# spaceandtimefdn/blitzar

Hardware: NVIDIA H100
Metric: MSM throughput (scalar*point terms/sec), ristretto255, n=2^20 per GPU (higher is better)
Workload: dtype u32 limbs (integer modular arithmetic)

## Files before the change

blitzar_b200/csrc/msm.cuh:

```cuda
#pragma once
#include <algorithm>
#include <vector>

#include "batch_affine.cuh"
#include "curve.cuh"
#include "engine_api.cuh"
#include "lanefield.cuh"

namespace b200 {

struct ColumnDesc {
  const unsigned char* base;
  u64 row_stride;
  u32 bit_offset;
  u32 bit_width;
  u32 n;
  u32 is_signed;
  u32 first_window;
  u32 num_windows;
  u32 table_n;
  u32 gen_base;
};
B200_HD u32 bucket_windows(const ColumnDesc& col) { return col.table_n ? (col.num_windows ? 1u : 0u) : col.num_windows; }

// ... 832 lines not shown
    typename F::E prefix[kMaxTableWindows], acc = F::one(), inv;
    C::gen_to_point(p, table[i], false);
    for (u32 w = 0; w < W; ++w) {
      if (w)
        for (u32 k = 0; k < c; ++k)
          C::dbl(p, p);
      pts[w] = p;
      prefix[w] = acc;
      F::mul(acc, acc, C::denominator(p));
    }
    F::invert(inv, acc);
    for (u32 w = W; w-- > 0;) {
      typename F::E zi;
      F::mul(zi, inv, prefix[w]);
      F::mul(inv, inv, C::denominator(pts[w]));
      typename C::Gen g;
      C::normalized_gen(g, pts[w], zi);
      table[(u64)w * n + i] = g;
    }
  }
};
template <class C> struct IngestCompactBody {
  static constexpr int kBlock = 128;
  const unsigned char* table;
  u32 window_width;
  typename C::Gen* gens;
  B200_HD void operator()(u64 i) const {
    const u64 group = i / window_width, j = i % window_width;
    const u64 entry = (group << window_width) + (1ull << j);
    typename C::Gen g;
    C::load_compact_abi(g, table + entry * C::kAbiCompactBytes);
    gens[i] = g;
  }
};
struct BuiltinGeneratorBody {
  static constexpr int kBlock = 64;
  Ed25519::Gen* gens;
  u64 first;
  B200_HD void operator()(u64 i) const {
    Ed25519::Point g;
    Ed25519::builtin_generator(g, first + i);
    Ed25519::point_to_gen(gens[i], g);
  }
};
struct GenPieces {
  const u64* start;
  const u64* from;
  const u64* to;
  u32 npieces;
};
template <class C> struct IngestPiecesBody {
  static constexpr int kBlock = IngestBody<C, false>::kBlock;
  const unsigned char* raw;
  typename C::Gen* gens;
  GenPieces p;
  B200_HD void operator()(u64 tid) const {
    const u32 k = column_of(p.start, p.npieces, tid);
    IngestBody<C, false>{raw + p.from[k] * C::kAbiGenBytes, gens + p.to[k]}(tid - p.start[k]);
  }
};
struct BuiltinPiecesBody {
  static constexpr int kBlock = BuiltinGeneratorBody::kBlock;
  Ed25519::Gen* gens;
  GenPieces p;
  B200_HD void operator()(u64 tid) const {
    const u32 k = column_of(p.start, p.npieces, tid);
    BuiltinGeneratorBody{gens + p.to[k], p.from[k]}(tid - p.start[k]);
  }
};

struct IngestMap {
  GenPieces p;
  B200_HD void at(u64 i, u64& src, u64& dst) const {
    if (p.npieces == 0) {
      src = dst = i;
      return;
    }
    const u32 k = column_of(p.start, p.npieces, i);
    src = p.from[k] + (i - p.start[k]);
    dst = p.to[k] + (i - p.start[k]);
  }
};
constexpr u32 kNormBlock = 256;
struct NormalizeUpBody {
  static constexpr int kBlock = 128;
  typedef F25519 F;
  const unsigned char* raw;
  IngestMap map;
  u64 n, T;
  F::E* pre;
  F::E* prod;
  u32* invalid;
  B200_HD F::E group(u64 j) const {
    F::E z[kBatchGroup], acc = F::one();
#pragma unroll
    for (u32 k = 0; k < kBatchGroup; ++k) {
      const u64 i = j + k * T;
      z[k] = F::one();
      if (i < n) {
        u64 src, dst;
        map.at(i, src, dst);
        z[k] = Ed25519::load_abi_z(raw + src * Ed25519::kAbiGenBytes);
      }
    }
#pragma unroll
    for (u32 k = 0; k < kBatchGroup; ++k) {
      const u64 i = j + k * T;
      if (i >= n)
        break;
      if (F::is_zero(z[k])) {
        *invalid = 1u;
        z[k] = F::one();
      }
      pre[i] = acc;
      F::mul(acc, acc, z[k]);
    }
    return acc;
  }
  B200_HD void operator()(u64 j) const { prod[j] = group(j); }
};
struct NormalizeDownBody {
  static constexpr int kBlock = 128;
  typedef F25519 F;
  const unsigned char* raw;
  IngestMap map;
  u64 n, T;
  const F::E* pre;
  const F::E* prod;
  const F::E* ps;
  const u32* invalid;
  Ed25519::Gen* gens;
  B200_HD void operator()(u64 j) const {
    const bool scale = *invalid == 0;
    F::E inv = prod[ps ? j / kNormBlock : j];
    if (ps)
      F::mul(inv, inv, ps[j]);
    for (u32 k = kBatchGroup; k-- > 0;) {
      const u64 i = j + k * T;
      if (i >= n)
        continue;
      u64 src, dst;
      map.at(i, src, dst);
      Ed25519::Point p;
      Ed25519::load_point_abi(p, raw + src * Ed25519::kAbiGenBytes);
      if (scale) {
        F::E zi;
        F::mul(zi, inv, pre[i]);
        F::mul(inv, inv, p.Z);
        F::mul(p.X, p.X, zi);
        F::mul(p.Y, p.Y, zi);
        F::mul(p.T, p.T, zi);
        p.Z = F::one();
      }
      Ed25519::Gen g;
      Ed25519::point_to_gen(g, p);
      gens[dst] = g;
    }
  }
};
#ifdef B200_BINNED_SORT
__device__ __forceinline__ F25519::E shfl_up_fe(const F25519::E& a, u32 d) {
  F25519::E r;
#pragma unroll
  for (int k = 0; k < 8; ++k)
    r.l[k] = __shfl_up_sync(0xffffffffu, a.l[k], d);
  return r;
}
__device__ __forceinline__ F25519::E shfl_down_fe(const F25519::E& a, u32 d) {
  F25519::E r;
#pragma unroll
  for (int k = 0; k < 8; ++k)
    r.l[k] = __shfl_down_sync(0xffffffffu, a.l[k], d);
  return r;
}
template <int kBlock>
__device__ void block_prefix_suffix(const F25519::E& x, F25519::E& P, F25519::E& S,
                                    F25519::E& total, F25519::E* ws) {
  typedef F25519 F;
  const u32 lane = threadIdx.x & 31u, warp = threadIdx.x >> 5;
  F::E inc = x, sinc = x;
#pragma unroll
  for (u32 d = 1; d < 32; d <<= 1) {
    const F::E y = shfl_up_fe(inc, d), z = shfl_down_fe(sinc, d);
    if (lane >= d)
      F::mul(inc, inc, y);
    if (lane + d < 32)
      F::mul(sinc, sinc, z);
  }
  F::E pe = shfl_up_fe(inc, 1), se = shfl_down_fe(sinc, 1);
  if (lane == 0)
    pe = F::one();
  if (lane == 31) {
    se = F::one();
    ws[warp] = inc;
  }
  __syncthreads();
  F::E before = F::one(), after = F::one();
  for (u32 w = 0; w < kBlock / 32; ++w) {
    if (w < warp)
      F::mul(before, before, ws[w]);
    else if (w > warp)
      F::mul(after, after, ws[w]);
  }
  F::mul(P, before, pe);
  F::mul(S, se, after);
  F::mul(total, before, ws[warp]);
  F::mul(total, total, after);
  __syncthreads();
}
struct NormalizeUpBlockBody {
  static constexpr int kBlock = kNormBlock;
  typedef F25519 F;
  NormalizeUpBody up;
  F::E* ps;
  F::E* prod;
  __device__ void run(u32 b, unsigned char*) const {
    __shared__ F::E ws[kBlock / 32];
    const u64 j = (u64)b * kBlock + threadIdx.x;
    const F::E g = j < up.T ? up.group(j) : F::one();
    F::E P, S, total;
    block_prefix_suffix<kBlock>(g, P, S, total, ws);
    if (j < up.T)
      F::mul(ps[j], P, S);
    if (threadIdx.x == 0)
      prod[b] = total;
  }
};
struct NormalizeMidBody {
  static constexpr int kBlock = 1024;
  typedef F25519 F;
  F::E* vals;
  F::E* pre;
  u64 m;
  __device__ void run(u32, unsigned char*) const {
    __shared__ F::E ws[kBlock / 32];
    __shared__ F::E inv_total;
    const u64 per = (m + kBlock - 1) / kBlock, lo = min((u64)threadIdx.x * per, m),
              hi = min(lo + per, m);
    F::E c = F::one();
    for (u64 k = lo; k < hi; ++k) {
      pre[k] = c;
      F::mul(c, c, vals[k]);
    }
    F::E P, S, total;
    block_prefix_suffix<kBlock>(c, P, S, total, ws);
    if (threadIdx.x == 0)
      F::invert(inv_total, total);
    __syncthreads();
    F::E inv;
    F::mul(inv, inv_total, P);
    F::mul(inv, inv, S);
    for (u64 k = hi; k-- > lo;) {
      const F::E v = vals[k];
      F::mul(vals[k], inv, pre[k]);
      F::mul(inv, inv, v);
    }
  }
};
#endif
inline void ingest_normalized(stream_t s, const unsigned char* raw, Ed25519::Gen* gens,
                              const IngestMap& map, u64 n, u32* invalid) {
  typedef F25519::E fe;
  if (n == 0)
    return;
  const u64 T = (n + kBatchGroup - 1) / kBatchGroup;
  fe* pre = (fe*)dev_alloc(n * sizeof(fe), s);
  const NormalizeUpBody up{raw, map, n, T, pre, nullptr, invalid};
#ifdef B200_BINNED_SORT
  const u64 blocks = (T + kNormBlock - 1) / kNormBlock;
  fe* ps = (fe*)dev_alloc((T + 2 * blocks) * sizeof(fe), s);
  fe* prod = ps + T;
  launch_blocks(NormalizeUpBlockBody{up, ps, prod}, blocks, 0, s);
  launch_blocks(NormalizeMidBody{prod, prod + blocks, blocks}, 1, 0, s);
  launch(NormalizeDownBody{raw, map, n, T, pre, prod, ps, invalid, gens}, T, s);
  dev_free(ps, s);
#else
  fe* prod = (fe*)dev_alloc(T * sizeof(fe), s);
  NormalizeUpBody u = up;
  u.prod = prod;
  launch(u, T, s);
  batch_invert<F25519>(s, prod, T);
  launch(NormalizeDownBody{raw, map, n, T, pre, prod, nullptr, invalid, gens}, T, s);
  dev_free(prod, s);
#endif
  dev_free(pre, s);
}
template <class C, bool kCommit> struct StoreBody {
  static constexpr int kBlock = 32;
  const typename C::Point* pts;
  unsigned char* out;
  B200_HD void operator()(u64 i) const {
    if (kCommit)
      C::store_commit_abi(out + i * C::kAbiCommitBytes, pts[i]);
    else
      C::store_proj_abi(out + i * C::kAbiProjBytes, pts[i]);
  }
};
template <class C>
inline void launch_store_commit(stream_t s, const typename C::Point* pts, unsigned char* out,
                                u64 count, bool lane_tail) {
#ifdef B200_LANE_TAIL
  if constexpr (C::kCurveId == kRistretto255) {
    if (lane_tail && count && count <= 4096) {
      launch(StoreLaneBody{pts, out, count}, (count + 2) / 3 * 32, s);
      return;
    }
  }
#endif
  launch(StoreBody<C, true>{pts, out}, count, s);
}
template <class C> struct GenToProjBody {
  static constexpr int kBlock = 64;
  const typename C::Gen* gens;
  unsigned char* out;
  B200_HD void operator()(u64 i) const {
    typename C::Point p;
    C::gen_to_point(p, gens[i], false);
    C::store_proj_abi(out + i * C::kAbiProjBytes, p);
  }
};
template <class C> struct SumPartsBody {
  static constexpr int kBlock = 32;
  const typename C::Point* parts;
  u32 nparts, count;
  typename C::Point* out;
  B200_HD void operator()(u64 j) const {
    typename C::Point acc = parts[j];
    for (u32 r = 1; r < nparts; ++r)
      C::add(acc, acc, parts[(u64)r * count + j]);
    out[j] = acc;
  }
};

inline u32 choose_window_bits(u64 max_n, u32 max_width, u32 ncols, size_t point_bytes) {
  const double kMaxBucketBytes = 3.0e9;
  u32 best = 2;
  double best_cost = 1e300;
  for (u32 c = 2; c <= 16; ++c) {
    double W = (double)(max_width / c + 1);
    if (c > 8 && W * (double)(1u << (c - 1)) * (double)ncols * (double)point_bytes > kMaxBucketBytes)
      break;
    double cost = W * ((double)max_n + 2.5 * (double)(1u << (c - 1)));
    if (cost < best_cost) {
      best_cost = cost;
      best = c;
    }
  }
  return best;
}

struct MsmPlan {
  u32 c = 0, nbuckets = 0, ncols = 0, total_windows = 0;
  u64 nkeys = 0, max_n = 0, total_terms = 0, total_entries = 0;
  std::vector<ColumnDesc> cols;
};

inline MsmPlan msm_make_plan(std::vector<ColumnDesc> cols, const MsmOptions& opt,
                             size_t point_bytes) {
  MsmPlan p;
  p.ncols = (u32)cols.size();
  u32 max_width = 1;
  for (auto& col : cols) {
    p.max_n = std::max<u64>(p.max_n, col.n);
    p.total_terms += col.n;
    if (col.n)
      max_width = std::max(max_width, col.bit_width);
  }
  p.c = opt.window_bits ? opt.window_bits
                        : choose_window_bits(p.max_n, max_width, p.ncols, point_bytes);
  p.nbuckets = 1u << (p.c - 1);
  u64 max_entries = 0;
  for (auto& col : cols) {
    col.first_window = p.total_windows;
    col.num_windows = col.n ? col.bit_width / p.c + 1 : 0;
    p.total_windows += bucket_windows(col);
    max_entries += (u64)col.n * col.num_windows;
    if (col.table_n)
      B200_REQUIRE((u64)col.table_n * col.num_windows < (1ull << 31), "generator table too large");
    if (col.n)
      B200_REQUIRE((u64)col.gen_base + col.n + (u64)(col.num_windows - 1) * col.table_n < (1ull << 31),
                   "generator index of a column too large");
  }
  p.nkeys = (u64)p.total_windows * p.nbuckets;
  p.total_entries = max_entries;
  B200_REQUIRE(p.nkeys < (1ull << 32), "too many buckets for one pass");
  p.cols = std::move(cols);
  return p;
}

struct StagedRange {
  const ColumnDesc* d_cols = nullptr;
  const u64* d_col_start = nullptr;
  u64 total_terms = 0, max_entries = 0;
  u32 max_windows = 0;
  StagedRange(stream_t s, const MsmPlan& plan, u64 begin, u64 end) {
    const u32 ncols = plan.ncols;
    std::vector<ColumnDesc> cols(plan.cols);
    std::vector<u64> col_start(ncols + 1, 0);
    for (u32 j = 0; j < ncols; ++j) {
      u64 lo = std::min<u64>(begin, cols[j].n), hi = std::min<u64>(end, cols[j].n);
      cols[j].base += lo * cols[j].row_stride;
      cols[j].n = (u32)(hi - lo);
      col_start[j + 1] = col_start[j] + cols[j].n;
      max_entries += (u64)cols[j].n * cols[j].num_windows;
      max_windows = std::max(max_windows, cols[j].n ? cols[j].num_windows : 0u);
    }
    total_terms = col_start[ncols];
    if (total_terms == 0)
      return;
    B200_REQUIRE(max_entries < (1ull << 32) && end - begin < (1ull << 31),
                 "too many (term, window) entries for one sort pass");
    const size_t desc_bytes = ncols * sizeof(ColumnDesc), start_bytes = (ncols + 1) * sizeof(u64);
    std::vector<unsigned char> stage(desc_bytes + start_bytes);
    std::memcpy(stage.data(), cols.data(), desc_bytes);
    std::memcpy(stage.data() + desc_bytes, col_start.data(), start_bytes);
    d_cols = (const ColumnDesc*)stage_to_device(s, stage.data(), stage.size());
    d_col_start = (const u64*)((const unsigned char*)d_cols + desc_bytes);
  }
};

struct SortedLayout {
  u64* entries;
  u32* counts;
  u32* starts;
  u32* d_m;
  u64 slots_max;
  bool binned;
  BucketOffsets offsets() const { return {counts, starts}; }
};

inline SortedLayout sort_entries(stream_t s, const MsmPlan& plan, const StagedRange& r, u32 L,
                                 const MsmOptions& opt, u32* window_used) {
  const u32 ncols = plan.ncols, c = plan.c, nbuckets = plan.nbuckets;
  const u64 nkeys = plan.nkeys, max_entries = r.max_entries, total_terms = r.total_terms;
  SortedLayout out{};
  out.slots_max = L ? ((max_entries + nkeys * ((1ull << L) - 1) + (1ull << L) - 1) >> L) << L : max_entries;
  out.counts = (u32*)dev_alloc((nkeys + 1) * sizeof(u32), s);
  out.d_m = (u32*)dev_alloc(16 * sizeof(u32), s);
  out.entries = (u64*)dev_alloc(out.slots_max * sizeof(u64), s);
#ifdef B200_BINNED_SORT
  out.binned = L == 0 && opt.sort_path != 0 && binned_sort_shift(nkeys) <= kMaxBinShift &&
               (opt.sort_path == 2 || max_entries >= kBinnedSortMinEntries);
  if (out.binned)
    binned_sort(s, r.d_cols, r.d_col_start, ncols, c, nbuckets, total_terms, max_entries,
                r.max_windows, nkeys, out.entries, out.counts, out.d_m);
#endif
  if (!out.binned) {
    dev_zero(out.counts, (nkeys + 1) * sizeof(u32), s);
    launch(CountBody{r.d_cols, r.d_col_start, ncols, c, nbuckets, out.counts}, total_terms, s);
    if (L)
      launch(PadCountsBody{out.counts, (1u << L) - 1u}, nkeys, s);
    exclusive_scan(out.counts, nkeys + 1, s);
    copy_d2d(out.d_m, out.counts + nkeys, sizeof(u32), s);
    if (L) {
      out.starts = (u32*)dev_alloc((nkeys + 1) * sizeof(u32), s);
      copy_d2d(out.starts, out.counts, (nkeys + 1) * sizeof(u32), s);
    }
    const bool window_major = opt.scatter_window_major && r.max_windows > 1;
    launch(ScatterBody{r.d_cols, r.d_col_start, ncols, c, nbuckets, out.counts, out.entries,
                       window_major ? total_terms : 0},
           window_major ? total_terms * r.max_windows : total_terms, s);
  }
  if (L)
    launch(FillPadsBody{out.starts, out.counts, out.entries}, nkeys, s);
  launch(WindowUsedBody{out.offsets(), nbuckets, window_used}, plan.total_windows, s);
  return out;
}

inline unsigned sort_selftest(stream_t s, std::vector<ColumnDesc> cols, u32 c) {
  MsmOptions opt;
  opt.window_bits = c;
  const MsmPlan plan = msm_make_plan(std::move(cols), opt, 160);
  const StagedRange r(s, plan, 0, plan.max_n);
  if (r.total_terms == 0)
    return ~0u;
  const u64 nkeys = plan.nkeys, M = r.max_entries;
  DevBuf<u32> window_used(plan.total_windows, s);
  opt.sort_path = 0;
  const SortedLayout a = sort_entries(s, plan, r, 0, opt, window_used.p);
  opt.sort_path = 2;
  const SortedLayout b = sort_entries(s, plan, r, 0, opt, window_used.p);
  std::vector<u32> ca(nkeys + 1), cb(nkeys + 1), m(1);
  std::vector<u64> ea(M), eb(M);
  copy_d2h(ca.data(), a.counts, (nkeys + 1) * sizeof(u32), s);
  copy_d2h(cb.data(), b.counts, (nkeys + 1) * sizeof(u32), s);
  copy_d2h(m.data(), b.d_m, sizeof(u32), s);
  copy_d2h(ea.data(), a.entries, M * sizeof(u64), s);
  copy_d2h(eb.data(), b.entries, M * sizeof(u64), s);
  stream_sync(s);
  for (void* p : {(void*)a.entries, (void*)a.counts, (void*)a.d_m, (void*)b.entries, (void*)b.counts,
                  (void*)b.d_m, (void*)r.d_cols})
    dev_free(p, s);
  if (!b.binned)
    return ~0u;
  unsigned bad = m[0] == ca[nkeys] ? 0u : 1u;
  for (u64 k = 0; k < nkeys; ++k) {
    const u32 lo = k ? ca[k - 1] : 0u, hi = ca[k];
    if (cb[k] != hi || hi < lo || hi > M) {
      ++bad;
      continue;
    }
    std::sort(ea.begin() + lo, ea.begin() + hi);
    std::sort(eb.begin() + lo, eb.begin() + hi);
    if (!std::equal(ea.begin() + lo, ea.begin() + hi, eb.begin() + lo))
      ++bad;
  }
  return bad;
}

struct RangeHook {
  virtual void before_range(u64 begin, u64 end) = 0;
  virtual void before_accumulate() {}
  virtual ~RangeHook() {}
};

template <class C>
stream_t chunk_walk(stream_t s, stream_t tail, WalkInput<C> walk, u32* d_m, bool unit,
                    const u32* unit_veto, typename C::Point* target, const MsmOptions& opt,
                    std::vector<void*>& to_free) {
  typedef typename C::Point Point;
  u32 K = opt.chunk1 ? std::max(opt.chunk1, 4u) : (walk.m_max >= (1ull << 23) ? 64u : 32u);
  const u32 chunkn = std::max(opt.chunkn, 4u);
  const u32* lvl_keys = nullptr;
  const Point* lvl_pieces = nullptr;
  stream_t cs = s;
  for (int level = 0;; ++level) {
    const bool final_level = walk.m_max <= K;
    u64 T = (walk.m_max + K - 1) / K;
    u32* out_keys = final_level ? nullptr : (u32*)dev_alloc(2 * T * sizeof(u32), cs);
    Point* out_pieces = final_level ? nullptr : (Point*)dev_alloc(2 * T * sizeof(Point), cs);
    to_free.insert(to_free.end(), {out_keys, out_pieces});
    u32* out_m = d_m + 1 + (level % 8);
    const auto launch_level = [&](auto body, u64 threads, stream_t st) {
      body = {lvl_keys, walk.entries, walk.gens, lvl_pieces, walk.m_ptr, K, final_level, target,
              out_keys, out_pieces, out_m, unit_veto};
      launch(body, threads, st);
    };
    if (level == 0) {
      const bool uniform =
          opt.uniform_add == 2 ? C::kCurveId == kRistretto255 : opt.uniform_add != 0;
      constexpr bool kEd = C::kCurveId == kRistretto255;
      const bool unit_path = kEd && unit;
      if (uniform && unit_path)
        launch_level(AccumulateBody<C, true, SeqExec, true, kEd>{}, T, s);
      else if (uniform)
        launch_level(AccumulateBody<C, true, SeqExec, true>{}, T, s);
      else if (unit_path)
        launch_level(AccumulateBody<C, true, SeqExec, false, kEd>{}, T, s);
      else
        launch_level(AccumulateBody<C, true>{}, T, s);
      KernelTimer::get().end(s);
      if (tail != s)
        stream_follow(tail, s);
      cs = tail;
    } else if (T <= opt.quad_threshold) {
      launch_level(AccumulateBody<C, false, QuadExec>{}, T * QuadExec::kLanes, cs);
    } else {
      launch_level(AccumulateBody<C, false>{}, T, cs);
    }
    if (final_level)
      break;
    lvl_keys = out_keys;
    lvl_pieces = out_pieces;
    walk.m_ptr = out_m;
    walk.m_max = 2 * T;
    K = chunkn;
  }
  return cs;
}

template <class C>
void msm_accumulate_range(stream_t s, const MsmPlan& plan, const typename C::Gen* gens, u64 begin,
                          u64 end, bool add_into, typename C::Point* d_buckets,
                          u32* d_window_used, const MsmOptions& opt, stream_t tail,
                          RangeHook* hook = nullptr) {
  const StagedRange r(s, plan, begin, end);
  if (r.total_terms == 0)
    return;
  gens += begin;
  StageRange nvtx_sort("msm: digit count + scan + scatter");
  const u64 max_entries = r.max_entries, nkeys = plan.nkeys;
  u32 L = 0;
  if constexpr (C::kBatchAffine) {
    const double mean = (double)max_entries / (double)nkeys;
    if (opt.pair_levels >= 0)
      L = (u32)opt.pair_levels;
    else if (max_entries >= (1ull << 23))
      while (L < 6 && (double)(32u << L) <= mean)
        ++L;
    while (L > 0 && max_entries + nkeys * ((1ull << L) - 1) >= (1ull << 32) - (1ull << L))
      --L;
  }
  const SortedLayout sorted = sort_entries(s, plan, r, L, opt, d_window_used);
  B200_LOG(3, "range [%llu, %llu): %llu terms, %llu entries max, c=%u, %llu keys, pair levels %u",
           (unsigned long long)begin, (unsigned long long)end, (unsigned long long)r.total_terms,
           (unsigned long long)max_entries, plan.c, (unsigned long long)nkeys, L);
  WalkInput<C> walk{gens, sorted.entries, sorted.d_m, max_entries};
  std::vector<void*> to_free;
  if (hook)
    hook->before_accumulate();
  KernelTimer::get().begin(s);
  StageRange nvtx_acc("msm: bucket accumulation");
  if constexpr (C::kBatchAffine) {
    if (L) {
      walk = run_pair_levels<C>(s, L, sorted.entries, gens, sorted.d_m, sorted.slots_max,
                                opt.pair_batch);
      to_free = {(void*)walk.gens, (void*)walk.entries};
    }
  }
  typedef typename C::Point Point;
  Point* target = add_into ? (Point*)dev_alloc(nkeys * sizeof(Point), s) : d_buckets;
  const bool unit = walk.gens == gens && opt.gens_normalized;
  const stream_t cs =
      chunk_walk<C>(s, tail, walk, sorted.d_m, unit, opt.unit_veto, target, opt, to_free);
  if (add_into) {
    launch(MergeBucketsBody<C>{sorted.offsets(), target, d_buckets}, nkeys, cs);
    dev_free(target, cs);
  }
  to_free.insert(to_free.end(), {sorted.d_m, sorted.counts, sorted.starts});
  for (void* ptr : to_free)
    dev_free(ptr, cs);
  dev_free(sorted.entries, s);
  dev_free((void*)r.d_cols, s);
}

template <class C>
void msm_finish(stream_t s, const MsmPlan& plan, const typename C::Point* d_buckets,
                const u32* d_window_used, typename C::Point* out, const MsmOptions& opt) {
  typedef typename C::Point Point;
  StageRange nvtx_fin("msm: bucket reduction + window combination");
  const u32 total_windows = plan.total_windows, nbuckets = plan.nbuckets, ncols = plan.ncols;
  ColumnDesc* d_cols =
      (ColumnDesc*)stage_to_device(s, plan.cols.data(), ncols * sizeof(ColumnDesc));
  Point* d_S = nullptr;
  u32 m = nbuckets;
  const Point* X = d_buckets;
  const Point* Cin = nullptr;
  std::vector<void*> to_free;
  if (m == 1) {
    d_S = (Point*)dev_alloc(total_windows * sizeof(Point), s);
    copy_d2d(d_S, d_buckets, total_windows * sizeof(Point), s);
  }
  bool first = true;
  while (m > 1) {
    u32 g = first ? std::min<u32>(opt.reduce_g1, m) : std::min<u32>(opt.reduce_gn, m);
    u32 log2g = 0;
    while ((1u << log2g) < g)
      ++log2g;
    u32 m_out = m / g;
    Point* Xout = (Point*)dev_alloc((u64)total_windows * m_out * sizeof(Point), s);
    Point* Cout = (Point*)dev_alloc((u64)total_windows * m_out * sizeof(Point), s);
    if ((u64)total_windows * m_out <= opt.quad_threshold)
      launch(ReduceBody<C, QuadExecConv>{X, Cin, m, g, log2g, Xout, Cout, d_window_used, nbuckets},
             (u64)total_windows * m_out * QuadExec::kLanes, s);
    else
      launch(ReduceBody<C>{X, Cin, m, g, log2g, Xout, Cout, d_window_used, nbuckets},
             (u64)total_windows * m_out, s);
    to_free.push_back(Xout);
    if (m_out > 1)
      to_free.push_back(Cout);
    X = Xout;
    Cin = Cout;
    m = m_out;
    first = false;
    if (m == 1)
      d_S = Cout;
  }
  for (void* ptr : to_free)
    dev_free(ptr, s);
  bool uniform_windows = true;
  for (u32 j = 1; j < ncols; ++j)
    uniform_windows = uniform_windows && bucket_windows(plan.cols[j]) == bucket_windows(plan.cols[0]);
#ifdef B200_LANE_TAIL
  bool lane_done = false;
  if constexpr (C::kCurveId == kRistretto255) {
    if (ncols <= 2048 && opt.lane_tail) {
      launch(CombineLaneBody{d_S, d_cols, plan.c, out}, (u64)ncols * 32, s);
      lane_done = true;
    }
  }
  if (lane_done) {
  } else
#endif
  if (ncols <= opt.quad_threshold && uniform_windows)
    launch(CombineBody<C, QuadExecConv>{d_S, d_cols, plan.c, out}, (u64)ncols * QuadExec::kLanes,
           s);
  else if (ncols <= opt.quad_threshold)
    launch(CombineBody<C, QuadExec>{d_S, d_cols, plan.c, out}, (u64)ncols * QuadExec::kLanes, s);
  else
    launch(CombineBody<C>{d_S, d_cols, plan.c, out}, ncols, s);
  dev_free(d_S, s);
  dev_free(d_cols, s);
}

template <class C>
void msm_run(stream_t s, const typename C::Gen* gens, std::vector<ColumnDesc> cols,
             typename C::Point* out, const MsmOptions& opt = MsmOptions(), u32 num_ranges = 1,
             RangeHook* hook = nullptr, stream_t tail = stream_t()) {
  typedef typename C::Point Point;
  if (cols.empty())
    return;
  MsmPlan plan = msm_make_plan(std::move(cols), opt, sizeof(Point));
  B200_LOG(2, "msm: curve %u, %u columns, longest %llu, %llu terms, window %u bits, %u bucket sets%s",
           C::kCurveId, plan.ncols, (unsigned long long)plan.max_n,
           (unsigned long long)plan.total_terms, plan.c, plan.total_windows,
           plan.ncols && plan.cols[0].table_n ? " (fixed-base table)" : "");
  if (plan.total_terms == 0 || plan.total_windows == 0) {
    if (hook)
      hook->before_range(0, plan.max_n);
    fill_identity<C>(s, out, plan.ncols);
    return;
  }
  Point* d_buckets = (Point*)dev_alloc(plan.nkeys * sizeof(Point), s);
  fill_identity<C>(s, d_buckets, plan.nkeys);
  u32* d_window_used = (u32*)dev_alloc(plan.total_windows * sizeof(u32), s);
  dev_zero(d_window_used, plan.total_windows * sizeof(u32), s);
  if (num_ranges < 1)
    num_ranges = 1;
  const u64 limit = opt.max_range_entries ? opt.max_range_entries : (1ull << 31);
  const u64 needed = (plan.total_entries + limit - 1) / limit;
  if (needed > num_ranges)
    num_ranges = (u32)std::min<u64>(needed, plan.max_n);
  const bool overlap = num_ranges > 1 && tail != stream_t() && tail != s;
  for (u32 r = 0; r < num_ranges; ++r) {
    u64 begin = range_begin(plan.max_n, r, num_ranges, opt.range_skew),
        end = range_begin(plan.max_n, r + 1, num_ranges, opt.range_skew);
    if (hook)
      hook->before_range(begin, end);
    msm_accumulate_range<C>(s, plan, gens, begin, end, r > 0, d_buckets, d_window_used, opt,
                            overlap ? tail : s, hook);
  }
  if (overlap)
    stream_follow(s, tail);
  msm_finish<C>(s, plan, d_buckets, d_window_used, out, opt);
  dev_free(d_window_used, s);
  dev_free(d_buckets, s);
}

}
```

blitzar_b200/csrc/runtime.cuh:

```cuda
#pragma once
#include <cstdio>
#include <cstdlib>
#include <cstring>
#include <atomic>
#include <cctype>
#include <string>
#include <utility>
#include <vector>

#include "field.cuh"

#ifndef B200_EMULATE
#include <cuda_runtime.h>
#include <nvtx3/nvToolsExt.h>
#endif

namespace b200 {

[[noreturn]] inline void die(const char* what, const char* file, int line) {
  std::fprintf(stderr, "blitzar_b200: fatal: %s (%s:%d)\n", what, file, line);
  std::abort();
}
#define B200_REQUIRE(cond, msg)                                                                    \
  do {                                                                                             \
    if (!(cond))                                                                                   \
      ::b200::die(msg, __FILE__, __LINE__);                                                        \
  } while (0)

inline int log_level() {
  static const int level = [] {
    const char* env = std::getenv("BLITZAR_LOG_LEVEL");
    if (!env)
      return 0;
    std::string s(env);
    for (auto& ch : s)
      ch = (char)std::tolower((unsigned char)ch);
    if (s == "warn")
      return 1;
    if (s == "info")
      return 2;
    if (s == "debug" || s == "trace")
      return 3;
    return 0;
  }();
  return level;
}
#define B200_LOG(level, ...)                                                                       \
  do {                                                                                             \
    if (::b200::log_level() >= (level)) {                                                          \
      std::fprintf(stderr, "[blitzar_b200] " __VA_ARGS__);                                         \
      std::fputc('\n', stderr);                                                                    \
    }                                                                                              \
  } while (0)

struct StageRange {
#ifndef B200_EMULATE
  explicit StageRange(const char* name) { nvtxRangePushA(name); }
  ~StageRange() { nvtxRangePop(); }
#else
  explicit StageRange(const char*) {}
#endif
  StageRange(const StageRange&) = delete;
  StageRange& operator=(const StageRange&) = delete;
};

#ifndef B200_EMULATE
#define B200_CUDA(call)                                                                            \
  do {                                                                                             \
    cudaError_t e_ = (call);                                                                       \
    if (e_ != cudaSuccess)                                                                         \
      ::b200::die(cudaGetErrorString(e_), __FILE__, __LINE__);                                     \
  } while (0)

typedef cudaStream_t stream_t;

template <class Body, class = void> struct MinBlocks {
  static constexpr int value = 1;
};
template <class Body> struct MinBlocks<Body, decltype((void)Body::kMinBlocks)> {
  static constexpr int value = Body::kMinBlocks;
};
template <class Body>
__global__ void __launch_bounds__(Body::kBlock, MinBlocks<Body>::value) k_run(Body body, u64 n) {
  u64 tid = (u64)blockIdx.x * blockDim.x + threadIdx.x;
  if (tid < n)
    body(tid);
}

struct LaunchCounter {
  static std::atomic<unsigned long long>& value() {
    static std::atomic<unsigned long long> v{0};
    return v;
  }
};

template <class Body> inline void launch(const Body& body, u64 n, stream_t s) {
  if (n == 0)
    return;
  u64 blocks = (n + Body::kBlock - 1) / Body::kBlock;
  B200_REQUIRE(blocks < (1ull << 31), "grid too large");
  k_run<Body><<<(unsigned)blocks, Body::kBlock, 0, s>>>(body, n);
  B200_CUDA(cudaGetLastError());
  ++LaunchCounter::value();
}
template <class Body> __global__ void __launch_bounds__(Body::kBlock) k_block(Body body) {
  extern __shared__ __align__(16) unsigned char smem[];
  body.run(blockIdx.x, smem);
}
template <class Body>
inline void launch_blocks(const Body& body, u64 blocks, size_t smem_bytes, stream_t s) {
  if (blocks == 0)
    return;
  B200_REQUIRE(blocks < (1ull << 31), "grid too large");
  static thread_local size_t raised = 48 * 1024;
  if (smem_bytes > raised) {
    B200_CUDA(cudaFuncSetAttribute(k_block<Body>, cudaFuncAttributeMaxDynamicSharedMemorySize,
                                   (int)smem_bytes));
    raised = smem_bytes;
  }
  k_block<Body><<<(unsigned)blocks, Body::kBlock, smem_bytes, s>>>(body);
  B200_CUDA(cudaGetLastError());
  ++LaunchCounter::value();
}
inline void* dev_alloc(size_t bytes, stream_t s) {
  void* p = nullptr;
  B200_CUDA(cudaMallocAsync(&p, bytes ? bytes : 16, s));
  return p;
}
inline void dev_free(void* p, stream_t s) {
  if (p)
    B200_CUDA(cudaFreeAsync(p, s));
}
inline void dev_zero(void* p, size_t bytes, stream_t s) { B200_CUDA(cudaMemsetAsync(p, 0, bytes, s)); }
inline void copy_h2d(void* d, const void* h, size_t bytes, stream_t s) {
  if (bytes)
    B200_CUDA(cudaMemcpyAsync(d, h, bytes, cudaMemcpyHostToDevice, s));
}
inline void copy_d2h(void* h, const void* d, size_t bytes, stream_t s) {
  if (bytes)
    B200_CUDA(cudaMemcpyAsync(h, d, bytes, cudaMemcpyDeviceToHost, s));
}
inline void copy_d2d(void* d, const void* s_, size_t bytes, stream_t s) {
  if (bytes)
    B200_CUDA(cudaMemcpyAsync(d, s_, bytes, cudaMemcpyDeviceToDevice, s));
}
inline void stream_sync(stream_t s) { B200_CUDA(cudaStreamSynchronize(s)); }
inline void stream_follow(stream_t later, stream_t earlier) {
  static thread_local cudaEvent_t ring[64];
  static thread_local unsigned next = 0;
  cudaEvent_t& e = ring[next++ % 64];
  if (!e)
    B200_CUDA(cudaEventCreateWithFlags(&e, cudaEventDisableTiming));
  B200_CUDA(cudaEventRecord(e, earlier));
  B200_CUDA(cudaStreamWaitEvent(later, e, 0));
}

inline stream_t aux_stream() {
  static thread_local cudaStream_t s = nullptr;
  if (!s)
    B200_CUDA(cudaStreamCreateWithFlags(&s, cudaStreamNonBlocking));
  return s;
}

struct StagingRing {
  static constexpr size_t kSlotBytes = 65536, kSlots = 128;
  unsigned char* base = nullptr;
  cudaEvent_t done[kSlots];
  size_t next = 0;
  static StagingRing& get() {
    static thread_local StagingRing r;
    return r;
  }
  void* stage(stream_t s, const void* host, size_t bytes) {
    void* d = dev_alloc(bytes, s);
    if (bytes > kSlotBytes) {
      copy_h2d(d, host, bytes, s);
      stream_sync(s);
      return d;
    }
    if (!base) {
      B200_CUDA(cudaHostAlloc((void**)&base, kSlotBytes * kSlots, cudaHostAllocDefault));
      for (auto& e : done) {
        B200_CUDA(cudaEventCreateWithFlags(&e, cudaEventDisableTiming));
      }
    }
    size_t slot = next++ % kSlots;
    B200_CUDA(cudaEventSynchronize(done[slot]));
    std::memcpy(base + slot * kSlotBytes, host, bytes);
    B200_CUDA(cudaMemcpyAsync(d, base + slot * kSlotBytes, bytes, cudaMemcpyHostToDevice, s));
    B200_CUDA(cudaEventRecord(done[slot], s));
    return d;
  }
};
inline void* stage_to_device(stream_t s, const void* host, size_t bytes) {
  return StagingRing::get().stage(s, host, bytes);
}

struct KernelTimer {
  bool enabled = false;
  std::vector<std::pair<cudaEvent_t, cudaEvent_t>> spans;
  static KernelTimer& get() {
    static thread_local KernelTimer t;
    return t;
  }
  void begin(stream_t s) {
    if (!enabled)
      return;
    cudaEvent_t a, b;
    B200_CUDA(cudaEventCreate(&a));
    B200_CUDA(cudaEventCreate(&b));
    B200_CUDA(cudaEventRecord(a, s));
    spans.emplace_back(a, b);
  }
  void end(stream_t s) {
    if (!enabled)
      return;
    B200_CUDA(cudaEventRecord(spans.back().second, s));
  }
  void read(float* total_ms, unsigned* count) {
    float tot = 0;
    for (auto& sp : spans) {
      float ms = 0;
      B200_CUDA(cudaEventSynchronize(sp.second));
      B200_CUDA(cudaEventElapsedTime(&ms, sp.first, sp.second));
      tot += ms;
      B200_CUDA(cudaEventDestroy(sp.first));
      B200_CUDA(cudaEventDestroy(sp.second));
    }
    *total_ms = tot;
    *count = (unsigned)spans.size();
    spans.clear();
  }
};
template <class T> B200_HD T atomic_add(T* p, T v) {
#ifdef __CUDA_ARCH__
  return atomicAdd(p, v);
#else
  T old = *p;
  *p = old + v;
  return old;
#endif
}
#define B200_ATOMIC_ADD(ptr, v) ::b200::atomic_add((ptr), (v))
#else
typedef int stream_t;
struct LaunchCounter {
  static unsigned long long& value() {
    static unsigned long long v = 0;
    return v;
  }
};
template <class Body> inline void launch(const Body& body, u64 n, stream_t) {
  for (u64 t = 0; t < n; ++t)
    body(t);
  ++LaunchCounter::value();
}
inline void* dev_alloc(size_t bytes, stream_t) { return std::malloc(bytes ? bytes : 16); }
inline void dev_free(void* p, stream_t) { std::free(p); }
inline void dev_zero(void* p, size_t bytes, stream_t) { std::memset(p, 0, bytes); }
inline void copy_h2d(void* d, const void* h, size_t bytes, stream_t) { std::memcpy(d, h, bytes); }
inline void copy_d2h(void* h, const void* d, size_t bytes, stream_t) { std::memcpy(h, d, bytes); }
inline void copy_d2d(void* d, const void* s_, size_t bytes, stream_t) { std::memcpy(d, s_, bytes); }
inline void stream_sync(stream_t) {}
inline void stream_follow(stream_t, stream_t) {}
inline stream_t aux_stream() { return 0; }
inline void* stage_to_device(stream_t s, const void* host, size_t bytes) {
  void* d = dev_alloc(bytes, s);
  std::memcpy(d, host, bytes);
  return d;
}
struct KernelTimer {
  static KernelTimer& get() {
    static KernelTimer t;
    return t;
  }
  void begin(stream_t) {}
  void end(stream_t) {}
};
template <class T> inline T emul_atomic_add(T* p, T v) {
  T old = *p;
  *p = old + v;
  return old;
}
#define B200_ATOMIC_ADD(ptr, v) ::b200::emul_atomic_add((ptr), (v))
#endif

}
```

Measured before the change: 350.9 million.

## Chain tail kernels with programmatic dependent launch and preallocate level buffers

Adds a chained launch path that sets the programmatic stream serialization attribute and has every kernel execute griddepcontrol.wait at entry. This lets the next kernel's launch overlap the previous one's tail in the bucket-walk, reduction, combine and store stages. Intermediate level buffers and the column descriptors are now allocated up front rather than between launches, so no async alloc or free sits between chained kernels. Because no kernel issues an explicit launch_dependents trigger, the overlap is limited to launch latency, and buffer lifetimes grow slightly.

```diff
diff --git a/blitzar_b200/csrc/msm.cuh b/blitzar_b200/csrc/msm.cuh
--- a/blitzar_b200/csrc/msm.cuh
+++ b/blitzar_b200/csrc/msm.cuh
@@ -1158,12 +1158,12 @@
 #ifdef B200_LANE_TAIL
   if constexpr (C::kCurveId == kRistretto255) {
     if (lane_tail && count && count <= 4096) {
-      launch(StoreLaneBody{pts, out, count}, (count + 2) / 3 * 32, s);
+      launch(StoreLaneBody{pts, out, count}, (count + 2) / 3 * 32, s, true);
       return;
     }
   }
 #endif
-  launch(StoreBody<C, true>{pts, out}, count, s);
+  launch(StoreBody<C, true>{pts, out}, count, s, true);
 }
 template <class C> struct GenToProjBody {
   static constexpr int kBlock = 64;
@@ -1380,17 +1380,24 @@
   const u32* lvl_keys = nullptr;
   const Point* lvl_pieces = nullptr;
   stream_t cs = s;
+  std::vector<std::pair<u32*, Point*>> outs;
+  for (u64 m = walk.m_max, k = K; m > k; k = chunkn) {
+    const u64 T = (m + k - 1) / k;
+    outs.push_back({(u32*)dev_alloc(2 * T * sizeof(u32), s),
+                    (Point*)dev_alloc(2 * T * sizeof(Point), s)});
+    to_free.insert(to_free.end(), {outs.back().first, outs.back().second});
+    m = 2 * T;
+  }
   for (int level = 0;; ++level) {
     const bool final_level = walk.m_max <= K;
     u64 T = (walk.m_max + K - 1) / K;
-    u32* out_keys = final_level ? nullptr : (u32*)dev_alloc(2 * T * sizeof(u32), cs);
-    Point* out_pieces = final_level ? nullptr : (Point*)dev_alloc(2 * T * sizeof(Point), cs);
-    to_free.insert(to_free.end(), {out_keys, out_pieces});
+    u32* out_keys = final_level ? nullptr : outs[level].first;
+    Point* out_pieces = final_level ? nullptr : outs[level].second;
     u32* out_m = d_m + 1 + (level % 8);
     const auto launch_level = [&](auto body, u64 threads, stream_t st) {
       body = {lvl_keys, walk.entries, walk.gens, lvl_pieces, walk.m_ptr, K, final_level, target,
               out_keys, out_pieces, out_m, unit_veto};
-      launch(body, threads, st);
+      launch(body, threads, st, true);
     };
     if (level == 0) {
       const bool uniform =
@@ -1470,7 +1477,7 @@
   const stream_t cs =
       chunk_walk<C>(s, tail, walk, sorted.d_m, unit, opt.unit_veto, target, opt, to_free);
   if (add_into) {
-    launch(MergeBucketsBody<C>{sorted.offsets(), target, d_buckets}, nkeys, cs);
+    launch(MergeBucketsBody<C>{sorted.offsets(), target, d_buckets}, nkeys, cs, true);
     dev_free(target, cs);
   }
   to_free.insert(to_free.end(), {sorted.d_m, sorted.counts, sorted.starts});
@@ -1482,12 +1489,11 @@
 
 template <class C>
 void msm_finish(stream_t s, const MsmPlan& plan, const typename C::Point* d_buckets,
-                const u32* d_window_used, typename C::Point* out, const MsmOptions& opt) {
+                const u32* d_window_used, const ColumnDesc* d_cols, typename C::Point* out,
+                const MsmOptions& opt) {
   typedef typename C::Point Point;
   StageRange nvtx_fin("msm: bucket reduction + window combination");
   const u32 total_windows = plan.total_windows, nbuckets = plan.nbuckets, ncols = plan.ncols;
-  ColumnDesc* d_cols =
-      (ColumnDesc*)stage_to_device(s, plan.cols.data(), ncols * sizeof(ColumnDesc));
   Point* d_S = nullptr;
   u32 m = nbuckets;
   const Point* X = d_buckets;
@@ -1497,21 +1503,30 @@
     d_S = (Point*)dev_alloc(total_windows * sizeof(Point), s);
     copy_d2d(d_S, d_buckets, total_windows * sizeof(Point), s);
   }
+  const auto group = [&](u32 m, bool first) {
+    return first ? std::min<u32>(opt.reduce_g1, m) : std::min<u32>(opt.reduce_gn, m);
+  };
+  std::vector<Point*> level_out;
+  for (u32 k = m; k > 1; k /= group(k, k == m)) {
+    const u64 bytes = (u64)total_windows * (k / group(k, k == m)) * sizeof(Point);
+    level_out.push_back((Point*)dev_alloc(bytes, s));
+    level_out.push_back((Point*)dev_alloc(bytes, s));
+  }
   bool first = true;
-  while (m > 1) {
-    u32 g = first ? std::min<u32>(opt.reduce_g1, m) : std::min<u32>(opt.reduce_gn, m);
+  for (u32 level = 0; m > 1; ++level) {
+    u32 g = group(m, first);
     u32 log2g = 0;
     while ((1u << log2g) < g)
       ++log2g;
     u32 m_out = m / g;
-    Point* Xout = (Point*)dev_alloc((u64)total_windows * m_out * sizeof(Point), s);
-    Point* Cout = (Point*)dev_alloc((u64)total_windows * m_out * sizeof(Point), s);
+    Point* Xout = level_out[2 * level];
+    Point* Cout = level_out[2 * level + 1];
     if ((u64)total_windows * m_out <= opt.quad_threshold)
       launch(ReduceBody<C, QuadExecConv>{X, Cin, m, g, log2g, Xout, Cout, d_window_used, nbuckets},
-             (u64)total_windows * m_out * QuadExec::kLanes, s);
+             (u64)total_windows * m_out * QuadExec::kLanes, s, true);
     else
       launch(ReduceBody<C>{X, Cin, m, g, log2g, Xout, Cout, d_window_used, nbuckets},
-             (u64)total_windows * m_out, s);
+             (u64)total_windows * m_out, s, true);
     to_free.push_back(Xout);
     if (m_out > 1)
       to_free.push_back(Cout);
@@ -1522,8 +1537,6 @@
     if (m == 1)
       d_S = Cout;
   }
-  for (void* ptr : to_free)
-    dev_free(ptr, s);
   bool uniform_windows = true;
   for (u32 j = 1; j < ncols; ++j)
     uniform_windows = uniform_windows && bucket_windows(plan.cols[j]) == bucket_windows(plan.cols[0]);
@@ -1531,7 +1544,7 @@
   bool lane_done = false;
   if constexpr (C::kCurveId == kRistretto255) {
     if (ncols <= 2048 && opt.lane_tail) {
-      launch(CombineLaneBody{d_S, d_cols, plan.c, out}, (u64)ncols * 32, s);
+      launch(CombineLaneBody{d_S, d_cols, plan.c, out}, (u64)ncols * 32, s, true);
       lane_done = true;
     }
   }
@@ -1540,13 +1553,15 @@
 #endif
   if (ncols <= opt.quad_threshold && uniform_windows)
     launch(CombineBody<C, QuadExecConv>{d_S, d_cols, plan.c, out}, (u64)ncols * QuadExec::kLanes,
-           s);
+           s, true);
   else if (ncols <= opt.quad_threshold)
-    launch(CombineBody<C, QuadExec>{d_S, d_cols, plan.c, out}, (u64)ncols * QuadExec::kLanes, s);
+    launch(CombineBody<C, QuadExec>{d_S, d_cols, plan.c, out}, (u64)ncols * QuadExec::kLanes, s,
+           true);
   else
-    launch(CombineBody<C>{d_S, d_cols, plan.c, out}, ncols, s);
+    launch(CombineBody<C>{d_S, d_cols, plan.c, out}, ncols, s, true);
+  for (void* ptr : to_free)
+    dev_free(ptr, s);
   dev_free(d_S, s);
-  dev_free(d_cols, s);
 }
 
 template <class C>
@@ -1568,6 +1583,8 @@
     return;
   }
   Point* d_buckets = (Point*)dev_alloc(plan.nkeys * sizeof(Point), s);
+  const ColumnDesc* d_cols =
+      (const ColumnDesc*)stage_to_device(s, plan.cols.data(), plan.ncols * sizeof(ColumnDesc));
   fill_identity<C>(s, d_buckets, plan.nkeys);
   u32* d_window_used = (u32*)dev_alloc(plan.total_windows * sizeof(u32), s);
   dev_zero(d_window_used, plan.total_windows * sizeof(u32), s);
@@ -1588,7 +1605,8 @@
   }
   if (overlap)
     stream_follow(s, tail);
-  msm_finish<C>(s, plan, d_buckets, d_window_used, out, opt);
+  msm_finish<C>(s, plan, d_buckets, d_window_used, d_cols, out, opt);
+  dev_free((void*)d_cols, s);
   dev_free(d_window_used, s);
   dev_free(d_buckets, s);
 }
diff --git a/blitzar_b200/csrc/runtime.cuh b/blitzar_b200/csrc/runtime.cuh
--- a/blitzar_b200/csrc/runtime.cuh
+++ b/blitzar_b200/csrc/runtime.cuh
@@ -80,8 +80,14 @@
 template <class Body> struct MinBlocks<Body, decltype((void)Body::kMinBlocks)> {
   static constexpr int value = Body::kMinBlocks;
 };
+__device__ __forceinline__ void chain_entry() {
+#if defined(__CUDA_ARCH__) && __CUDA_ARCH__ >= 900
+  asm volatile("griddepcontrol.wait;" ::: "memory");
+#endif
+}
 template <class Body>
 __global__ void __launch_bounds__(Body::kBlock, MinBlocks<Body>::value) k_run(Body body, u64 n) {
+  chain_entry();
   u64 tid = (u64)blockIdx.x * blockDim.x + threadIdx.x;
   if (tid < n)
     body(tid);
@@ -94,33 +100,51 @@
   }
 };
 
-template <class Body> inline void launch(const Body& body, u64 n, stream_t s) {
+template <class Kernel, class... Args>
+inline void launch_kernel(Kernel kernel, u64 blocks, unsigned block, size_t smem, stream_t s,
+                          bool chained, Args... args) {
+  B200_REQUIRE(blocks < (1ull << 31), "grid too large");
+  if (chained) {
+    cudaLaunchAttribute attr[1];
+    attr[0].id = cudaLaunchAttributeProgrammaticStreamSerialization;
+    attr[0].val.programmaticStreamSerializationAllowed = 1;
+    cudaLaunchConfig_t cfg = {};
+    cfg.gridDim = dim3((unsigned)blocks);
+    cfg.blockDim = dim3(block);
+    cfg.dynamicSmemBytes = smem;
+    cfg.stream = s;
+    cfg.attrs = attr;
+    cfg.numAttrs = 1;
+    B200_CUDA(cudaLaunchKernelEx(&cfg, kernel, args...));
+  } else {
+    kernel<<<(unsigned)blocks, block, smem, s>>>(args...);
+    B200_CUDA(cudaGetLastError());
+  }
+  ++LaunchCounter::value();
+}
+template <class Body> inline void launch(const Body& body, u64 n, stream_t s, bool chained = false) {
   if (n == 0)
     return;
-  u64 blocks = (n + Body::kBlock - 1) / Body::kBlock;
-  B200_REQUIRE(blocks < (1ull << 31), "grid too large");
-  k_run<Body><<<(unsigned)blocks, Body::kBlock, 0, s>>>(body, n);
-  B200_CUDA(cudaGetLastError());
-  ++LaunchCounter::value();
+  launch_kernel(k_run<Body>, (n + Body::kBlock - 1) / Body::kBlock, Body::kBlock, 0, s, chained,
+                body, n);
 }
 template <class Body> __global__ void __launch_bounds__(Body::kBlock) k_block(Body body) {
+  chain_entry();
   extern __shared__ __align__(16) unsigned char smem[];
   body.run(blockIdx.x, smem);
 }
 template <class Body>
-inline void launch_blocks(const Body& body, u64 blocks, size_t smem_bytes, stream_t s) {
+inline void launch_blocks(const Body& body, u64 blocks, size_t smem_bytes, stream_t s,
+                          bool chained = false) {
   if (blocks == 0)
     return;
-  B200_REQUIRE(blocks < (1ull << 31), "grid too large");
   static thread_local size_t raised = 48 * 1024;
   if (smem_bytes > raised) {
     B200_CUDA(cudaFuncSetAttribute(k_block<Body>, cudaFuncAttributeMaxDynamicSharedMemorySize,
                                    (int)smem_bytes));
     raised = smem_bytes;
   }
-  k_block<Body><<<(unsigned)blocks, Body::kBlock, smem_bytes, s>>>(body);
-  B200_CUDA(cudaGetLastError());
-  ++LaunchCounter::value();
+  launch_kernel(k_block<Body>, blocks, Body::kBlock, smem_bytes, s, chained, body);
 }
 inline void* dev_alloc(size_t bytes, stream_t s) {
   void* p = nullptr;
@@ -250,7 +274,7 @@
     return v;
   }
 };
-template <class Body> inline void launch(const Body& body, u64 n, stream_t) {
+template <class Body> inline void launch(const Body& body, u64 n, stream_t, bool = false) {
   for (u64 t = 0; t < n; ++t)
     body(t);
   ++LaunchCounter::value();
```

Result: no change. 353.3 million, median of 6 (+0.7%).
